# zrlhahaha/Direct12PBRRenderer

Measured on AMD Instinct MI355X. Metric: shaded Mpixel/s at 4K G-buffer (full deferred frame: clustered shade + bloom + auto-exposure + ACES), higher is better.
Workload: dtype f32

## Files before the change

### direct12pbrrenderer_amd/csrc/shade.hip

```cpp
#include <cstring>
#include <type_traits>
#include "pbr_internal.hpp"
#include "pbr_device.hpp"

using namespace pbr;

struct ShadeParams {
    pbr_sh_pack sh;
    float InvView[9];
    float CameraPos[3];
    float Near, Far;
    float near_width, near_height;
    float log_far_near;
    float inv_near, slice_k;
    uint32_t x0, y0, w, h, full_w, full_h;
    const uint32_t* A;
    const uint32_t* B;
    const uint32_t* C;
    const float* depth;
    const uint8_t* stencil;
    uint32_t pitch;
    const pbr_half* lut;
    uint32_t lut_res;
    const pbr_half* env;
    uint32_t env_size, env_mips;
    uint32_t env_mip_off[16];
    const pbr_cluster* clusters;
    const pbr_light* lights;
    pbr_half* hdr;
    uint32_t hdr_pitch;
    float* hdr_f32;
};

__device__ __forceinline__ float view_space_depth(float d, float near_z, float far_z) {
#pragma clang fp contract(off)
    const float range = far_z - near_z;
    const float prod = d * range;
    const float den = far_z - prod;
    const float num = near_z * far_z;
    return num / den;
}

__device__ __forceinline__ float view_space_depth_quick(float d, float near_z, float far_z) {
#pragma clang fp contract(off)
    const float range = far_z - near_z;
    const float prod = d * range;
    const float den = far_z - prod;
    return (near_z * far_z) * rcp(den);
}

__device__ __forceinline__ float sign_custom(float x) { return x < 0.0f ? -1.0f : 1.0f; }

__device__ __forceinline__ V3 decode_octahedron(float u, float v) {
    V3 d = v3(u * 2.0f - 1.0f, v * 2.0f - 1.0f, 0.0f);
    d.z = 1.0f - fabsf(d.x) - fabsf(d.y);
    if (d.z < 0.0f) {
// ... 31 lines not shown
struct ShadeRects {
    uint32_t n, rows_big, rows_small;
    uint32_t x0[SHADE_MAX_RECTS], y0[SHADE_MAX_RECTS], w[SHADE_MAX_RECTS], h[SHADE_MAX_RECTS];
    uint32_t cols[SHADE_MAX_RECTS], nb_big[SHADE_MAX_RECTS], first[SHADE_MAX_RECTS + 1];
};

constexpr int SHADE_BLOCK = 256;
constexpr int SHADE_ROWS = 8;
constexpr int MAX_STAGED_TILES = 12;
constexpr int LIST_STRIDE = 34;

typedef float f2 __attribute__((ext_vector_type(2)));
__device__ __forceinline__ f2 f2s(float a) { return f2{a, a}; }
__device__ __forceinline__ f2 max2(f2 a, f2 b) { return f2{fmaxf(a.x, b.x), fmaxf(a.y, b.y)}; }
typedef __attribute__((address_space(3))) const float lds_cf;
__device__ __forceinline__ f2 rsq2(f2 a) { return f2{rsq(a.x), rsq(a.y)}; }
__device__ __forceinline__ f2 rcp2(f2 a) { return f2{rcp(a.x), rcp(a.y)}; }

__device__ __forceinline__ f2 mul2_sat(f2 a, f2 b) {
    f2 r;
    asm("s_nop 0\n\tv_pk_mul_f32 %0, %1, %2 clamp\n\ts_nop 0" : "=v"(r) : "v"(a), "v"(b));
    return r;
}

__device__ __forceinline__ f2 zero2() {
    f2 r;
    asm("v_pk_mov_b32 %0, 0, 0\n\ts_nop 0" : "=v"(r));
    return r;
}

struct alignas(8) H4x2 { H4 a, b; };
struct alignas(4) H2x2 { H2 a, b; };

template <bool STAGED_LISTS, int LSTRIDE, bool F32OUT>
__device__ __forceinline__ void shade_pixel(const ShadeParams& p, const float* llds, const uint32_t* lists, const uint32_t* mip_off,
                                            int tile_x0, int tile_y0, int tiles_x, int n_lights, int q_safe, uint32_t px, uint32_t py, float4 row) {
    const uint32_t gi = __umul24(py, p.pitch) + px;
    auto at = [](const auto* base, uint32_t byte_off) { return *reinterpret_cast<std::remove_reference_t<decltype(*base)>*>(reinterpret_cast<const char*>(base) + byte_off); };
    if (at(p.stencil, gi) == 0) return;
    const float inv255 = 1.0f / 255.0f;

    const float u = ((float)(p.x0 + px) + 0.5f) / (float)p.full_w;
    V3 pos, view, n;
    float z_vs, roughness, depth_keep;
    {
        const uint32_t b = at(p.B, gi * 4u), c = at(p.C, gi * 4u);
        const float depth_ndc = at(p.depth, gi * 4u);
        const float ndc_x = 2.0f * u - 1.0f;
        const V3 cvv = v3(ndc_x * 0.5f * p.near_width, row.y, p.Near);
        const V3 camera_vec = v3(p.InvView[0] * cvv.x + p.InvView[1] * cvv.y + p.InvView[2] * cvv.z,
                                 p.InvView[3] * cvv.x + p.InvView[4] * cvv.y + p.InvView[5] * cvv.z,
                                 p.InvView[6] * cvv.x + p.InvView[7] * cvv.y + p.InvView[8] * cvv.z);
        roughness = (float)(c & 255u) * inv255;
        n = normalize3(decode_octahedron((float)(b & 255u) * inv255, (float)((b >> 8) & 255u) * inv255));
        z_vs = view_space_depth_quick(depth_ndc, p.Near, p.Far);
        depth_keep = depth_ndc;
        const V3 cam = v3(p.CameraPos[0], p.CameraPos[1], p.CameraPos[2]);
        const float zs = z_vs * p.inv_near;
        pos = v3(cam.x + camera_vec.x * zs, cam.y + camera_vec.y * zs, cam.z + camera_vec.z * zs);
        view = normalize3(cam - pos);
    }
    const float NdV = dot3(n, view);
    const float NdotV = fmaxf(NdV, 0.0f);

    float s1x = 0.0f, s1y = 0.0f, s1z = 0.0f, s2x = 0.0f, s2y = 0.0f, s2z = 0.0f, s3x = 0.0f, s3y = 0.0f, s3z = 0.0f;
#ifndef PBR_EXP_NOLOOP
    if (STAGED_LISTS || n_lights > 0) {
        int sx = (int)floorf(u * (float)PBR_CLUSTER_X);
        int sy = (int)row.z;
        float zc = fminf(fmaxf(z_vs, p.Near), p.Far);
        const float t_quick = p.slice_k * __builtin_amdgcn_logf(zc * p.inv_near);
        const float t_frac = t_quick - floorf(t_quick);
        int sz = (int)t_quick;
        if (__any(!(t_frac > 1.0e-4f && t_frac < 1.0f - 1.0e-4f))) {
            zc = fminf(fmaxf(view_space_depth(depth_keep, p.Near, p.Far), p.Near), p.Far);
            sz = (int)((float)PBR_CLUSTER_Z * logf(zc / p.Near) / p.log_far_near);
        }
        sx = clampi(sx, 0, PBR_CLUSTER_X - 1);
        sz = clampi(sz, 0, PBR_CLUSTER_Z - 1);
        const float ra = roughness * roughness;
        const float a4m1 = ra * ra - 1.0f;
        const float k = (roughness + 1.0f) * (roughness + 1.0f) * 0.125f;
        const float one_k = 1.0f - k;
        const float c4 = 4.0e4f * NdotV;
        const float t_floor = EPSILON_F * INV_PI_F;
        f2 a1x = zero2(), a1y = zero2(), a1z = zero2(), a2x = zero2(), a2y = zero2(), a2z = zero2(), a3x = zero2(), a3y = zero2(), a3z = zero2();
        const float att_c0 = llds[6 * LSTRIDE], att_c1 = llds[7 * LSTRIDE], att_c2 = llds[8 * LSTRIDE];
        auto light2 = [&](auto q_safe, auto t_safe, const lds_cf* la, const lds_cf* lb, auto att_uniform) {
            constexpr bool QSAFE = decltype(q_safe)::value, TSAFE = decltype(t_safe)::value, ATT = decltype(att_uniform)::value;
            auto comp = [&](int c) { return f2{la[c * LSTRIDE], lb[c * LSTRIDE]}; };
            const f2 dx = comp(0) - f2s(pos.x), dy = comp(1) - f2s(pos.y), dz = comp(2) - f2s(pos.z);
            const f2 d2 = dx * dx + dy * dy + dz * dz;
            const f2 invd = rsq2(d2);
            const f2 dn = dx * n.x + dy * n.y + dz * n.z;
            const f2 NdotL = mul2_sat(dn, invd);
            const f2 wx = dx * invd + f2s(view.x), wy = dy * invd + f2s(view.y), wz = dz * invd + f2s(view.z);
            const f2 h2 = wx * wx + (wy * wy + (wz * wz + f2s(1.0e-15f)));
            const f2 nw = dn * invd + f2s(NdV);
            const f2 tn = (nw * nw) * a4m1 + h2;
            const f2 h4 = h2 * h2;
            f2 Tn = tn * tn;
            if constexpr (!TSAFE) Tn = max2(Tn, h4 * t_floor);
            const f2 A = NdotL * one_k + f2s(k);
            f2 Q;
            if constexpr (ATT) Q = d2 * (invd * f2s(att_c1) + f2s(att_c2)) + f2s(att_c0);
            else Q = d2 * (invd * comp(7) + comp(8)) + comp(6);
            if constexpr (!QSAFE) Q = max2(Q, f2s(EPSILON_F));
            const f2 TA = Tn * A;
            const f2 r = rcp2(Q * TA);
            const f2 q = NdotL * r;
            const f2 X = q * TA;
            const f2 gs = mul2_sat(NdotL, f2s(c4));
            const f2 fm = f2s(1.0f) - NdotL;
            const f2 fm2 = fm * fm;
            const f2 f5 = fm2 * fm2 * fm;
            const f2 w2 = (q * gs) * h4;
            const f2 w1 = X - X * f5;
            const f2 w3 = w2 * f5;
            const f2 cr = comp(3), cg = comp(4), cb = comp(5);
            a1x += cr * w1; a1y += cg * w1; a1z += cb * w1;
            a2x += cr * w2; a2y += cg * w2; a2z += cb * w2;
            a3x += cr * w3; a3y += cg * w3; a3z += cb * w3;
        };
        const lds_cf* const ltab = (const lds_cf*)llds;
        if (STAGED_LISTS) {
            const uint32_t* my = lists + __mul24(__mul24(__mul24(sy - tile_y0, tiles_x) + (sx - tile_x0), PBR_CLUSTER_Z) + sz, LIST_STRIDE);
            const int nl = my[0];
            const bool t_ok = __all(ra * ra >= 6.0e-4f) != 0;
            auto walk = [&](auto qs, auto ts, auto au) {
                int i = 0;
                do {
                    const uint2 pair = *reinterpret_cast<const uint2*>(my + 2 + i);
                    light2(qs, ts, (const lds_cf*)(uintptr_t)pair.x, (const lds_cf*)(uintptr_t)pair.y, au);
                    i += 2;
                } while (i < nl);
            };
            if (q_safe & 1) {
                if (t_ok) { if (q_safe & 2) walk(std::true_type{}, std::true_type{}, std::true_type{}); else walk(std::true_type{}, std::true_type{}, std::false_type{}); }
                else if (q_safe & 2) walk(std::true_type{}, std::false_type{}, std::true_type{});
                else walk(std::true_type{}, std::false_type{}, std::false_type{});
            } else walk(std::false_type{}, std::false_type{}, std::false_type{});
        } else {
            const pbr_cluster* cl = p.clusters + (sz + sx * PBR_CLUSTER_Z + sy * PBR_CLUSTER_X * PBR_CLUSTER_Z);
            const int nl = min(max(cl->NumLights, 0), PBR_MAX_LIGHTS_PER_CLUSTER);
            auto idx = [&](int q) { return q < nl ? min(max(cl->LightIndex[q], 0), n_lights - 1) : n_lights; };
            for (int i = 0; i < nl; i += 2) light2(std::false_type{}, std::false_type{}, ltab + idx(i), ltab + idx(i + 1), std::false_type{});
        }
        s1x = a1x.x + a1x.y; s1y = a1y.x + a1y.y; s1z = a1z.x + a1z.y;
        s2x = a2x.x + a2x.y; s2y = a2y.x + a2y.y; s2z = a2z.x + a2z.y;
        s3x = a3x.x + a3x.y; s3y = a3y.x + a3y.y; s3z = a3z.x + a3z.y;
    }
#endif

    const uint32_t a = at(p.A, gi * 4u);
    const float metallic = (float)((at(p.C, gi * 4u) >> 8) & 255u) * inv255;
    const V3 albedo = v3((float)(a & 255u) * inv255, (float)((a >> 8) & 255u) * inv255, (float)((a >> 16) & 255u) * inv255);
    const float emission = (float)(a >> 24) * inv255;
    const V3 F0 = v3(0.04f + metallic * (albedo.x - 0.04f), 0.04f + metallic * (albedo.y - 0.04f), 0.04f + metallic * (albedo.z - 0.04f));
    V3 out;
    {
        const float ra = roughness * roughness;
        const float k = (roughness + 1.0f) * (roughness + 1.0f) * 0.125f;
        const float spec_pix = NdotV > 0.0f ? ra * ra * (0.25f * INV_PI_F) * rcp(fmaxf(NdotV * (1.0f - k) + k, EPSILON_F)) : 0.0f;
        const float kd = (1.0f - metallic) * INV_PI_F;
        out.x = (1.0f - F0.x) * (kd * albedo.x * s1x + spec_pix * s3x) + F0.x * spec_pix * s2x;
        out.y = (1.0f - F0.y) * (kd * albedo.y * s1y + spec_pix * s3y) + F0.y * spec_pix * s2y;
        out.z = (1.0f - F0.z) * (kd * albedo.z * s1z + spec_pix * s3z) + F0.z * spec_pix * s2z;
        out = out + albedo * emission;

#ifndef PBR_EXP_NOSH
        const float bx = n.x * n.y, by = n.y * n.z, bz = n.z * n.z, bw = n.z * n.x;
        const float cc = n.x * n.x - n.y * n.y;
        const pbr_sh_pack& s = p.sh;
        const float ir = (s.sha_r[0] * n.x + s.sha_r[1] * n.y + s.sha_r[2] * n.z + s.sha_r[3]) +
                         ((s.shb_r[0] * bx + s.shb_r[1] * by + s.shb_r[2] * bz + s.shb_r[3] * bw) + s.shc[0] * cc);
        const float ig = (s.sha_g[0] * n.x + s.sha_g[1] * n.y + s.sha_g[2] * n.z + s.sha_g[3]) +
                         ((s.shb_g[0] * bx + s.shb_g[1] * by + s.shb_g[2] * bz + s.shb_g[3] * bw) + s.shc[1] * cc);
        const float ib = (s.sha_b[0] * n.x + s.sha_b[1] * n.y + s.sha_b[2] * n.z + s.sha_b[3]) +
                         ((s.shb_b[0] * bx + s.shb_b[1] * by + s.shb_b[2] * bz + s.shb_b[3] * bw) + s.shc[2] * cc);
        out.x += albedo.x * kd * ir;
        out.y += albedo.y * kd * ig;
        out.z += albedo.z * kd * ib;
#endif
    }

#ifndef PBR_EXP_NOIBL
    {
#ifndef PBR_EXP_NOENV
        const V3 R = normalize3(n * (2.0f * NdV) - view);
        float lod = roughness * (float)PBR_ENV_MIPS;
        lod = snap8(fminf(fmaxf(lod, 0.0f), (float)(p.env_mips - 1)));
        const float fl = floorf(lod);
        const uint32_t l0 = (uint32_t)fl, l1 = min(l0 + 1, p.env_mips - 1);
        const float env_f = lod - fl;
        uint32_t face;
        float cu, cv;
        {
            const float ma = 0.5f * fabsf(__builtin_amdgcn_cubema(R.x, R.y, R.z));
            const float sc = __builtin_amdgcn_cubesc(R.x, R.y, R.z), tc = __builtin_amdgcn_cubetc(R.x, R.y, R.z);
            face = (uint32_t)__builtin_amdgcn_cubeid(R.x, R.y, R.z);
            const float inv = rcp(ma);
            cu = (sc * inv + 1.0f) * 0.5f;
            cv = (tc * inv + 1.0f) * 0.5f;
        }
        struct Foot { H4x2 r0, r1; float w00, w10, w01, w11; };
        auto foot = [&](uint32_t l, uint32_t mip_off, float wl) {
            const int s = (int)(p.env_size >> l), sq = s + 1;
            const float fxp = snap8(cu * (float)s) - 0.5f, fyp = snap8(cv * (float)s) - 0.5f;
            const float flx = floorf(fxp), fly = floorf(fyp);
            const float fx = fxp - flx, fy = fyp - fly;
            const uint32_t o = __umul24(__umul24(face, (uint32_t)sq) + (uint32_t)((int)fly + 1), (uint32_t)sq) + (uint32_t)((int)flx + 1);
            const char* q = reinterpret_cast<const char*>(p.env) + (mip_off + o * 4u) * 8u;
            Foot f;
            f.r0 = *reinterpret_cast<const H4x2*>(q);
            f.r1 = *reinterpret_cast<const H4x2*>(q + 16);
            const float wy1 = fy * wl, wy0 = wl - wy1;
            f.w10 = fx * wy0; f.w00 = wy0 - f.w10;
            f.w11 = fx * wy1; f.w01 = wy1 - f.w11;
            return f;
        };
        const Foot fa = foot(l0, mip_off[l0], 1.0f - env_f);
        const Foot fb = foot(l1, mip_off[l1], env_f);
        auto chan = [&](h16 a00, h16 a10, h16 a01, h16 a11, h16 b00, h16 b10, h16 b01, h16 b11) {
            float r = __builtin_fmaf((float)a00, fa.w00, 0.0f);
            r = __builtin_fmaf((float)a10, fa.w10, r);
            r = __builtin_fmaf((float)a01, fa.w01, r);
            r = __builtin_fmaf((float)a11, fa.w11, r);
            r = __builtin_fmaf((float)b00, fb.w00, r);
            r = __builtin_fmaf((float)b10, fb.w10, r);
            r = __builtin_fmaf((float)b01, fb.w01, r);
            return __builtin_fmaf((float)b11, fb.w11, r);
        };
        const V3 envc = v3(chan(fa.r0.a.x, fa.r0.b.x, fa.r1.a.x, fa.r1.b.x, fb.r0.a.x, fb.r0.b.x, fb.r1.a.x, fb.r1.b.x),
                           chan(fa.r0.a.y, fa.r0.b.y, fa.r1.a.y, fa.r1.b.y, fb.r0.a.y, fb.r0.b.y, fb.r1.a.y, fb.r1.b.y),
                           chan(fa.r0.a.z, fa.r0.b.z, fa.r1.a.z, fa.r1.b.z, fb.r0.a.z, fb.r0.b.z, fb.r1.a.z, fb.r1.b.z));
#else
        const V3 envc = v3(0.5f, 0.5f, 0.5f);
#endif
#ifndef PBR_EXP_NOLUT
        const int lr = (int)p.lut_res;
        const float lrf = (float)lr;
        const float xs = snap8(roughness * lrf) - 0.5f, ys = snap8(NdotV * lrf) - 0.5f;
        const float xfl = floorf(xs), yfl = floorf(ys);
        const int xi = (int)xfl, yi = (int)yfl;
        const int y0 = clampi(yi, 0, lr - 1), y1 = clampi(yi + 1, 0, lr - 1);
        const int xb = clampi(xi, 0, max(lr - 2, 0));
        const float fx = xi < 0 ? 0.0f : (xi > lr - 2 ? 1.0f : xs - xfl), fy = ys - yfl;
        const H2* lut = reinterpret_cast<const H2*>(p.lut);
        H2x2 lt0, lt1;
        if (lr > 1) {
            const char* lb8 = reinterpret_cast<const char*>(lut);
            lt0 = *reinterpret_cast<const H2x2*>(lb8 + (__umul24((uint32_t)y0, (uint32_t)lr) + (uint32_t)xb) * 4u);
            lt1 = *reinterpret_cast<const H2x2*>(lb8 + (__umul24((uint32_t)y1, (uint32_t)lr) + (uint32_t)xb) * 4u);
        } else {
            lt0.a = lt0.b = lut[0];
            lt1 = lt0;
        }
        const float wx0 = 1.0f - fx, wy0 = 1.0f - fy;
        auto xl = [&](h16 a, h16 b) { return __builtin_fmaf((float)b, fx, __builtin_fmaf((float)a, wx0, 0.0f)); };
        const float la = xl(lt0.a.x, lt0.b.x) * wy0 + xl(lt1.a.x, lt1.b.x) * fy;
        const float lb = xl(lt0.a.y, lt0.b.y) * wy0 + xl(lt1.a.y, lt1.b.y) * fy;
#else
        const float la = 0.5f, lb = 0.25f;
#endif
        out.x += envc.x * (F0.x * la + lb);
        out.y += envc.y * (F0.y * la + lb);
        out.z += envc.z * (F0.z * la + lb);
    }
#endif
    const uint32_t ho = __umul24(py, p.hdr_pitch) + px;
    if (F32OUT) *reinterpret_cast<float4*>(reinterpret_cast<char*>(p.hdr_f32) + ho * 16u) = make_float4(out.x, out.y, out.z, 1.0f);
    else store_h4(reinterpret_cast<pbr_half*>(reinterpret_cast<char*>(p.hdr) + ho * 8u), f4(out.x, out.y, out.z, 1.0f));
}

#ifdef PBR_SHADE_TIMING
__device__ unsigned long long g_shade_item_stamp[4 * 160000];
extern "C" int pbr_debug_shade_stamps(unsigned long long* blocks, int n_blocks, unsigned long long* items, int n_items) {
    (void)blocks; (void)n_blocks;
    return (int)hipMemcpyFromSymbol(items, HIP_SYMBOL(g_shade_item_stamp), sizeof(unsigned long long) * 4 * n_items);
}
extern "C" int pbr_debug_shade_stamps_reset() {
    void* i = nullptr;
    int e = (int)hipGetSymbolAddress(&i, HIP_SYMBOL(g_shade_item_stamp));
    if (e == 0) e = (int)hipMemset(i, 0, sizeof(g_shade_item_stamp));
    return e;
}
// ... 15 lines not shown
    const uint32_t* A;
    const uint32_t* B;
    const uint32_t* C;
    const float* depth;
    const uint8_t* stencil;
    const pbr_cluster* clusters;
    const pbr_light* lights;
    pbr_half* hdr;
    uint32_t pitch, hdr_pitch;
    int n_lights;
};
struct ShadeViews { ShadeView v[PBR_MAX_VIEWS]; };
static_assert(sizeof(ShadeParams) + sizeof(ShadeViews) + sizeof(ShadeRects) + 16 <= 4096 - 256, "k_deferred_shade<.., ShadeViews>: kernel arguments over 4 KiB");

template <bool STAGED_LISTS, int LSTRIDE, bool F32OUT, class VS = NoViews>
__global__ __launch_bounds__(SHADE_BLOCK, SHADE_MIN_WAVES) void k_deferred_shade(ShadeParams p_, int n_lights_, int max_clusters, ShadeRects rc, VS vs) {
    constexpr bool MV = !std::is_same_v<VS, NoViews>;
    ShadeParams q;
    int n_views_lights = 0;
    if constexpr (MV) {
        const ShadeView& v = vs.v[blockIdx.y];
        q = p_;
        for (int i = 0; i < 9; i++) q.InvView[i] = v.InvView[i];
        for (int i = 0; i < 3; i++) q.CameraPos[i] = v.CameraPos[i];
        q.Near = v.Near; q.Far = v.Far; q.near_width = v.near_width; q.near_height = v.near_height;
        q.log_far_near = v.log_far_near; q.inv_near = v.inv_near; q.slice_k = v.slice_k;
        q.A = v.A; q.B = v.B; q.C = v.C; q.depth = v.depth; q.stencil = v.stencil; q.pitch = v.pitch;
        q.clusters = v.clusters; q.lights = v.lights; q.hdr = v.hdr; q.hdr_pitch = v.hdr_pitch;
        n_views_lights = v.n_lights;
    }
    const ShadeParams& p = MV ? q : p_;
    const int n_lights = MV ? n_views_lights : n_lights_;
    extern __shared__ float4 lds_raw[];
    __shared__ uint32_t s_mip_off[16];
    const unsigned long long t_start = SHADE_NOW();
    (void)t_start;
    if (threadIdx.x < 16) s_mip_off[threadIdx.x] = p_.env_mip_off[threadIdx.x];
    float* llds = reinterpret_cast<float*>(lds_raw);
    uint32_t* lists = reinterpret_cast<uint32_t*>(llds + ((LIGHT_PLANES * LSTRIDE + 1) & ~1));
    int my_safe = 1, my_same = 1;
    const float att0 = n_lights > 0 ? p.lights[0].C0 : 1.0f, att1 = n_lights > 0 ? p.lights[0].C1 : 0.0f, att2 = n_lights > 0 ? p.lights[0].C2 : 0.0f;
    if (threadIdx.x == 0) {
        llds[0 * LSTRIDE + n_lights] = 1.0e15f; llds[1 * LSTRIDE + n_lights] = 1.0e15f; llds[2 * LSTRIDE + n_lights] = 1.0e15f;
        llds[3 * LSTRIDE + n_lights] = 0.0f; llds[4 * LSTRIDE + n_lights] = 0.0f; llds[5 * LSTRIDE + n_lights] = 0.0f;
        llds[6 * LSTRIDE + n_lights] = 1.0f; llds[7 * LSTRIDE + n_lights] = 0.0f; llds[8 * LSTRIDE + n_lights] = 0.0f;
    }
    for (int i = threadIdx.x; i < n_lights; i += SHADE_BLOCK) {
        const pbr_light l = p.lights[i];
        my_safe &= (l.C0 >= EPSILON_F) & (l.C1 >= 0.0f) & (l.C2 >= 0.0f);
        my_same &= (l.C0 == att0) & (l.C1 == att1) & (l.C2 == att2);
        llds[0 * LSTRIDE + i] = l.Position[0];
        llds[1 * LSTRIDE + i] = l.Position[1];
        llds[2 * LSTRIDE + i] = l.Position[2];
        llds[3 * LSTRIDE + i] = l.Color[0] * l.Intensity;
        llds[4 * LSTRIDE + i] = l.Color[1] * l.Intensity;
        llds[5 * LSTRIDE + i] = l.Color[2] * l.Intensity;
        llds[6 * LSTRIDE + i] = l.C0;
        llds[7 * LSTRIDE + i] = l.C1;
        llds[8 * LSTRIDE + i] = l.C2;
    }
    uint32_t r = 0;
    while (r + 1 < rc.n && blockIdx.x >= rc.first[r + 1]) r++;
    const uint32_t lb = blockIdx.x - rc.first[r];
    const uint32_t bx0 = rc.x0[r] + (lb % rc.cols[r]) * SHADE_BLOCK, x_end = rc.x0[r] + rc.w[r];
    const uint32_t by = lb / rc.cols[r], nb_big = rc.nb_big[r], rows_big = rc.rows_big, rows_small = rc.rows_small;
    const uint32_t y_begin = rc.y0[r] + (by < nb_big ? by * rows_big : nb_big * rows_big + (by - nb_big) * rows_small);
    const uint32_t y_end = min(y_begin + (by < nb_big ? rows_big : rows_small), rc.y0[r] + rc.h[r]);
    int tile_x0 = 0, tile_y0 = 0, tiles_x = 1;
    const uint32_t lds_base = (uint32_t)(uintptr_t)(lds_cf*)llds;
    if (STAGED_LISTS) {
        const uint32_t bx1 = min(bx0 + SHADE_BLOCK, x_end) - 1;
        auto tx = [&](uint32_t x) { return clampi((int)floorf((((float)(p.x0 + x) + 0.5f) / (float)p.full_w) * (float)PBR_CLUSTER_X), 0, PBR_CLUSTER_X - 1); };
// ... 11 lines not shown
            const int part = threadIdx.x & 7;
            const float inv_tiles_x = rcp((float)tiles_x);
            for (int c = threadIdx.x >> 3; c < n_cl; c += SHADE_BLOCK / 8) {
                const int z = c & 7, t = c >> 3;
                const int ty_ = (int)(((float)t + 0.5f) * inv_tiles_x), cx = tile_x0 + (t - ty_ * tiles_x), cy = tile_y0 + ty_;
                const pbr_cluster* cl = p.clusters + (z + cx * PBR_CLUSTER_Z + cy * PBR_CLUSTER_X * PBR_CLUSTER_Z);
                const int cnt = n_lights > 0 ? min(max(cl->NumLights, 0), PBR_MAX_LIGHTS_PER_CLUSTER) : 0;
                const Idx4 v = *reinterpret_cast<const Idx4*>(cl->LightIndex + 4 * part);
                uint32_t* l = lists + c * LIST_STRIDE;
                if (4 * part < max(cnt, 2)) {
                    auto entry = [&](int k, int raw) { return lds_base + 4u * (uint32_t)(4 * part + k < cnt ? min(max(raw, 0), n_lights - 1) : n_lights); };
                    uint2* e = reinterpret_cast<uint2*>(l + 2 + 4 * part);
                    e[0] = make_uint2(entry(0, v.x), entry(1, v.y));
                    e[1] = make_uint2(entry(2, v.z), entry(3, v.w));
                }
                if (part == 0) *reinterpret_cast<uint2*>(l) = make_uint2((uint32_t)max((cnt + 1) & ~1, 2), 0u);
            }
        }
    }
    __shared__ float4 s_row[SHADE_ROWS];
    if (threadIdx.x < (uint32_t)SHADE_ROWS) {
        const float v = ((float)(p.y0 + y_begin + threadIdx.x) + 0.5f) / (float)p.full_h;
        const float ndc_y = 1.0f - 2.0f * v;
        s_row[threadIdx.x] = make_float4(v, ndc_y * 0.5f * p.near_height, (float)clampi((int)floorf((1.0f - v) * (float)PBR_CLUSTER_Y), 0, PBR_CLUSTER_Y - 1), 0.0f);
    }
    const int q_safe = (__syncthreads_and(my_safe) != 0 ? 1 : 0) | (__syncthreads_and(my_same) != 0 ? 2 : 0);
    SHADE_ISTAMP(blockIdx.x, 0, t_start);
    SHADE_ISTAMP(blockIdx.x, 1, SHADE_NOW());
    SHADE_ISTAMP(blockIdx.x, 3, ((unsigned long long)(y_end - y_begin) << 48) | blockIdx.x);
    const uint32_t px = bx0 + threadIdx.x;
#ifndef PBR_SHADE_TIMING
    if (px >= x_end) return;
    for (uint32_t py = y_begin; py < y_end; py++)
        shade_pixel<STAGED_LISTS, LSTRIDE, F32OUT>(p, llds, lists, s_mip_off, tile_x0, tile_y0, tiles_x, n_lights, q_safe, px, py, s_row[py - y_begin]);
#else
    if (px < x_end)
        for (uint32_t py = y_begin; py < y_end; py++)
            shade_pixel<STAGED_LISTS, LSTRIDE, F32OUT>(p, llds, lists, s_mip_off, tile_x0, tile_y0, tiles_x, n_lights, q_safe, px, py, s_row[py - y_begin]);
    SHADE_ISTAMP_MAX(blockIdx.x, 2, SHADE_NOW());
#endif
}

extern "C" {

pbr_status pbr_env_pad(pbr_ctx* ctx, const pbr_half* env, uint32_t size, uint32_t mips, pbr_half* out_padded) {
    if (!ctx) return PBR_ERR_INVALID;
    PBR_REQUIRE(ctx, env && out_padded, "pbr_env_pad: null pointer");
    PBR_REQUIRE(ctx, size >= 1 && size <= 8192 && mips >= 1 && mips <= 16 && (size >> (mips - 1)) >= 1, "pbr_env_pad: bad size/mips");
    for (uint32_t m = 0; m < mips; m++) {
        const int s = (int)(size >> m);
        const size_t n = (size_t)6 * (s + 1) * (s + 1) * 4;
        hipLaunchKernelGGL(k_env_pad, dim3((unsigned)((n + 255) / 256)), dim3(256), 0, ctx->stream,
                           env + 4 * cube_mip_offset(size, m), out_padded + 4 * env_padded_mip_offset(size, m), s);
        pbr_status r = launched(ctx, "k_env_pad");
        if (r) return r;
    }
    return PBR_OK;
}

}

static void camera_params(const pbr_global* g, ShadeParams& p) {
    p.sh = g->SkyBoxSH;
    for (int r = 0; r < 3; r++)
        for (int c = 0; c < 3; c++) p.InvView[r * 3 + c] = g->InvView[r * 4 + c];
    for (int i = 0; i < 3; i++) p.CameraPos[i] = g->CameraPos[i];
    p.Near = g->Near; p.Far = g->Far;
    p.near_height = 2.0f * g->Near * tanf(g->Fov / 2.0f);
    p.near_width = p.near_height * g->Ratio;
    p.log_far_near = logf(g->Far / g->Near);
    p.inv_near = (float)(1.0 / (double)g->Near);
    p.slice_k = (float)((double)PBR_CLUSTER_Z / log2((double)g->Far / (double)g->Near));
}

static ShadeParams shade_params(const pbr_global* g, const pbr_half* lut, uint32_t lut_res, const pbr_half* env, uint32_t env_size, uint32_t env_mips) {
    ShadeParams p{};
    camera_params(g, p);
    p.lut = lut; p.lut_res = lut_res; p.env = env; p.env_size = env_size; p.env_mips = env_mips;
    for (uint32_t m = 0; m < 16; m++) p.env_mip_off[m] = (uint32_t)env_padded_mip_offset(env_size, m < env_mips ? m : env_mips - 1);
    return p;
}

static const char* shade_tables_bad(const pbr_half* lut, uint32_t lut_res, const pbr_half* env, uint32_t env_size, uint32_t env_mips) {
    if (!lut || !env) return "null pointer";
    if (!(lut_res >= 1 && env_size >= 1 && env_mips >= 1 && env_mips <= 16 && (env_size >> (env_mips - 1)) >= 1)) return "bad LUT/env size";
    if (!(lut_res <= 16384 && (uint64_t)pbr_env_padded_texels(env_size, env_mips) * 8u < (1ull << 32)))
        return "LUT larger than 16384^2 or padded env chain of 4 GiB or more (32-bit texture offsets)";
    if (((uintptr_t)env & 7u) != 0 || ((uintptr_t)lut & 3u) != 0) return "env must be 8-byte and lut 4-byte aligned";
    return nullptr;
}

static const char* shade_target_bad(const pbr_global* g, const pbr_gbuffer& gb, const pbr_cluster* clusters, const void* out, uint32_t out_pitch,
                                    uint32_t w, uint32_t h, const pbr_light* lights, int num_lights) {
    if (!clusters || !out) return "null pointer";
    if (!(gb.A && gb.B && gb.C && gb.depth && gb.stencil)) return "null G-buffer plane";
    if (!(gb.pitch >= w && out_pitch >= w)) return "pitch < width";
    if (!((uint64_t)gb.pitch * h * 4u < (1ull << 32) && (uint64_t)out_pitch * h * 16u < (1ull << 32)))
        return "target too large for 32-bit plane offsets (pitch x rows x 16 bytes must stay below 4 GiB)";
    if (!(g->Near > 0.0f && g->Far > g->Near)) return "need 0 < Near < Far";
    if (!(num_lights >= 0 && num_lights <= PBR_MAX_SCENE_LIGHTS)) return "light count out of [0, 1024]";
    if (!(num_lights == 0 || lights != nullptr)) return "null lights";
    return nullptr;
}

static ShadeRects shade_schedule(const pbr_ctx* ctx, const uint32_t (*rects)[4], uint32_t n_rects, uint32_t n_views) {
    static const float big_frac = pbr::knob_float("PBR_SHADE_BIGFRAC", 0.92f);
    static const uint32_t rows_small_cfg = (uint32_t)pbr::knob_int("PBR_SHADE_ROWS_SMALL", 1);
    static const uint32_t rows_big_cfg = (uint32_t)pbr::knob_int("PBR_SHADE_ROWS_BIG", 0);
    const uint32_t rows_small = rows_small_cfg >= 1 && rows_small_cfg <= (uint32_t)SHADE_ROWS ? rows_small_cfg : 1u;
    uint64_t row_segments = 0;
    for (uint32_t r = 0; r < n_rects; r++) row_segments += (uint64_t)((rects[r][2] + SHADE_BLOCK - 1) / SHADE_BLOCK) * rects[r][3];
    row_segments *= n_views;
    uint32_t rows_big = (uint32_t)SHADE_ROWS;
    const uint64_t slots = (uint64_t)ctx->cu_count * SHADE_MIN_WAVES;
    if (row_segments * 10 < slots * 13 * SHADE_ROWS) {
        const uint32_t rws = (uint32_t)((row_segments * 10 + slots * 8) / (slots * 16));
        rows_big = rws < 2 ? 2u : (rws > (uint32_t)SHADE_ROWS ? (uint32_t)SHADE_ROWS : rws);
    }
    if (rows_big_cfg >= 1 && rows_big_cfg <= (uint32_t)SHADE_ROWS) rows_big = rows_big_cfg;
    ShadeRects rc{};
    rc.n = n_rects; rc.rows_big = rows_big; rc.rows_small = rows_small < rows_big ? rows_small : rows_big;
    uint32_t blocks = 0;
    for (uint32_t r = 0; r < n_rects; r++) {
        const uint32_t* q = rects[r];
        rc.x0[r] = q[0]; rc.y0[r] = q[1]; rc.w[r] = q[2]; rc.h[r] = q[3];
        rc.cols[r] = (q[2] + SHADE_BLOCK - 1) / SHADE_BLOCK;
        rc.nb_big[r] = (uint32_t)((float)(q[3] / rows_big) * fminf(fmaxf(big_frac, 0.0f), 1.0f));
        const uint32_t rest = q[3] - rc.nb_big[r] * rows_big;
        rc.first[r] = blocks;
        blocks += rc.cols[r] * (rc.nb_big[r] + (rest + rc.rows_small - 1) / rc.rows_small);
    }
    rc.first[n_rects] = blocks;
    return rc;
}

template <bool F32OUT, class VS>
static pbr_status shade_dispatch(pbr_ctx* ctx, const ShadeParams& p, int num_lights, int max_lights, const ShadeRects& rc, uint32_t n_views, const VS& vs) {
    const uint32_t span_x = (uint32_t)((uint64_t)(SHADE_BLOCK - 1) * PBR_CLUSTER_X / p.full_w) + 2;
    const uint32_t span_y = (uint32_t)((uint64_t)(SHADE_ROWS - 1) * PBR_CLUSTER_Y / p.full_h) + 2;
    const int lstride = max_lights <= 256 ? 257 : PBR_MAX_SCENE_LIGHTS + 1;
    const size_t plane_bytes = (size_t)((LIGHT_PLANES * lstride + 1) & ~1) * sizeof(float);
    const bool staged = span_x * span_y <= (uint32_t)MAX_STAGED_TILES &&
                        plane_bytes + (size_t)span_x * span_y * PBR_CLUSTER_Z * LIST_STRIDE * sizeof(uint32_t) <= 65536;
    const int max_clusters = staged ? (int)(span_x * span_y) * PBR_CLUSTER_Z : 0;
    const size_t lds = plane_bytes + (size_t)max_clusters * LIST_STRIDE * sizeof(uint32_t);
    const dim3 grid(rc.first[rc.n], n_views), blk(SHADE_BLOCK);
    if (staged && lstride == 257) hipLaunchKernelGGL((k_deferred_shade<true, 257, F32OUT, VS>), grid, blk, lds, ctx->stream, p, num_lights, max_clusters, rc, vs);
    else if (staged) hipLaunchKernelGGL((k_deferred_shade<true, PBR_MAX_SCENE_LIGHTS + 1, F32OUT, VS>), grid, blk, lds, ctx->stream, p, num_lights, max_clusters, rc, vs);
    else if (lstride == 257) hipLaunchKernelGGL((k_deferred_shade<false, 257, F32OUT, VS>), grid, blk, lds, ctx->stream, p, num_lights, 0, rc, vs);
    else hipLaunchKernelGGL((k_deferred_shade<false, PBR_MAX_SCENE_LIGHTS + 1, F32OUT, VS>), grid, blk, lds, ctx->stream, p, num_lights, 0, rc, vs);
    return launched(ctx, std::is_same_v<VS, NoViews> ? "k_deferred_shade" : "k_deferred_shade<views>");
}

template <bool F32OUT>
static pbr_status shade_launch(pbr_ctx* ctx, const pbr_global* g, const pbr_tile* tile, const pbr_gbuffer* gb,
                               const pbr_half* lut, uint32_t lut_res,
                               const pbr_half* env, uint32_t env_size, uint32_t env_mips,
                               const pbr_cluster* clusters, const pbr_light* lights, int num_lights,
                               pbr_half* hdr, float* hdr_f32, uint32_t hdr_pitch,
                               const uint32_t (*rects)[4] = nullptr, uint32_t n_rects = 0) {
    if (!ctx) return PBR_ERR_INVALID;
    const char* who = "pbr_deferred_shade";
    PBR_REQUIRE(ctx, g && tile && gb, "pbr_deferred_shade: null pointer");
    PBR_REQUIRE(ctx, tile->w >= 1 && tile->h >= 1 && tile->w <= 65535 && tile->h <= 65535, "pbr_deferred_shade: bad tile size");
    PBR_REQUIRE(ctx, tile->x0 + tile->w <= tile->full_w && tile->y0 + tile->h <= tile->full_h, "pbr_deferred_shade: tile outside frame");
    PBR_CHECK(ctx, who, shade_target_bad(g, *gb, clusters, F32OUT ? (const void*)hdr_f32 : (const void*)hdr, hdr_pitch, tile->w, tile->h, lights, num_lights));
    PBR_CHECK(ctx, who, shade_tables_bad(lut, lut_res, env, env_size, env_mips));
    const uint32_t whole[1][4] = {{0, 0, tile->w, tile->h}};
    if (!rects) { rects = whole; n_rects = 1; }
    PBR_REQUIRE(ctx, n_rects >= 1 && n_rects <= (uint32_t)SHADE_MAX_RECTS, "pbr_deferred_shade: 1 .. 5 rectangles");
    for (uint32_t r = 0; r < n_rects; r++) {
        const uint32_t* q = rects[r];
        PBR_REQUIRE(ctx, q[2] >= 1 && q[3] >= 1 && q[0] + q[2] <= tile->w && q[1] + q[3] <= tile->h, "pbr_deferred_shade: rectangle outside the tile");
    }
    ShadeParams p = shade_params(g, lut, lut_res, env, env_size, env_mips);
    p.x0 = tile->x0; p.y0 = tile->y0; p.w = tile->w; p.h = tile->h; p.full_w = tile->full_w; p.full_h = tile->full_h;
    p.A = gb->A; p.B = gb->B; p.C = gb->C; p.depth = gb->depth; p.stencil = gb->stencil; p.pitch = gb->pitch;
    p.clusters = clusters; p.lights = lights; p.hdr = hdr; p.hdr_pitch = hdr_pitch; p.hdr_f32 = hdr_f32;
    return shade_dispatch<F32OUT>(ctx, p, num_lights, num_lights, shade_schedule(ctx, rects, n_rects, 1), 1, NoViews{});
}

extern "C" {

pbr_status pbr_deferred_shade(pbr_ctx* ctx, const pbr_global* g, const pbr_tile* tile, const pbr_gbuffer* gb,
                              const pbr_half* lut, uint32_t lut_res,
                              const pbr_half* env, uint32_t env_size, uint32_t env_mips,
                              const pbr_cluster* clusters, const pbr_light* lights, int num_lights,
                              pbr_half* hdr, uint32_t hdr_pitch) {
    return shade_launch<false>(ctx, g, tile, gb, lut, lut_res, env, env_size, env_mips, clusters, lights, num_lights, hdr, nullptr, hdr_pitch);
}

pbr_status pbr_deferred_shade_rects(pbr_ctx* ctx, const pbr_global* g, const pbr_tile* tile, const pbr_gbuffer* gb,
                                    const pbr_half* lut, uint32_t lut_res,
                                    const pbr_half* env, uint32_t env_size, uint32_t env_mips,
                                    const pbr_cluster* clusters, const pbr_light* lights, int num_lights,
                                    pbr_half* hdr, uint32_t hdr_pitch, const uint32_t (*rects)[4], uint32_t n_rects) {
    if (ctx && !rects) return pbr::fail(ctx, PBR_ERR_INVALID, "pbr_deferred_shade_rects: null rectangle list");
    return shade_launch<false>(ctx, g, tile, gb, lut, lut_res, env, env_size, env_mips, clusters, lights, num_lights, hdr, nullptr, hdr_pitch, rects, n_rects);
}

pbr_status pbr_deferred_shade_f32(pbr_ctx* ctx, const pbr_global* g, const pbr_tile* tile, const pbr_gbuffer* gb,
                                  const pbr_half* lut, uint32_t lut_res,
                                  const pbr_half* env, uint32_t env_size, uint32_t env_mips,
                                  const pbr_cluster* clusters, const pbr_light* lights, int num_lights,
                                  float* hdr_f32, uint32_t hdr_pitch) {
    if (ctx && hdr_f32 && ((uintptr_t)hdr_f32 & 15u) != 0) return pbr::fail(ctx, PBR_ERR_INVALID, "pbr_deferred_shade_f32: output must be 16-byte aligned");
    return shade_launch<true>(ctx, g, tile, gb, lut, lut_res, env, env_size, env_mips, clusters, lights, num_lights, nullptr, hdr_f32, hdr_pitch);
}

pbr_status pbr_deferred_shade_views(pbr_ctx* ctx, const pbr_view* views, uint32_t n, uint32_t w, uint32_t h,
                                    const pbr_half* lut, uint32_t lut_res,
                                    const pbr_half* env, uint32_t env_size, uint32_t env_mips) {
    if (!ctx) return PBR_ERR_INVALID;
    const char* who = "pbr_deferred_shade_views";
    PBR_REQUIRE(ctx, views_count_ok(views, n), "pbr_deferred_shade_views: need 1 .. PBR_MAX_VIEWS views");
    PBR_REQUIRE(ctx, w >= 1 && h >= 1 && w <= 65535 && h <= 65535, "pbr_deferred_shade_views: bad frame size");
    PBR_CHECK(ctx, who, shade_tables_bad(lut, lut_res, env, env_size, env_mips));
    ShadeViews vs{};
    int max_lights = 0;
    for (uint32_t i = 0; i < n; i++) {
        const pbr_view& v = views[i];
        PBR_CHECK(ctx, who, shade_target_bad(&v.g, v.gb, v.clusters, v.hdr, v.hdr_pitch, w, h, v.lights, v.num_lights));
        PBR_REQUIRE(ctx, memcmp(&v.g.SkyBoxSH, &views[0].g.SkyBoxSH, sizeof(pbr_sh_pack)) == 0, "pbr_deferred_shade_views: SkyBoxSH differs between views");
        ShadeParams c;
        camera_params(&v.g, c);
        ShadeView& d = vs.v[i];
        for (int k = 0; k < 9; k++) d.InvView[k] = c.InvView[k];
        for (int k = 0; k < 3; k++) d.CameraPos[k] = c.CameraPos[k];
        d.Near = c.Near; d.Far = c.Far; d.near_width = c.near_width; d.near_height = c.near_height;
        d.log_far_near = c.log_far_near; d.inv_near = c.inv_near; d.slice_k = c.slice_k;
        d.A = v.gb.A; d.B = v.gb.B; d.C = v.gb.C; d.depth = v.gb.depth; d.stencil = v.gb.stencil; d.pitch = v.gb.pitch;
        d.clusters = v.clusters; d.lights = v.lights; d.hdr = v.hdr; d.hdr_pitch = v.hdr_pitch; d.n_lights = v.num_lights;
        max_lights = v.num_lights > max_lights ? v.num_lights : max_lights;
    }
    PBR_REQUIRE(ctx, views_disjoint(views, n, 1, [&](const pbr_view& v, int, uintptr_t& lo, uintptr_t& hi) {
                    lo = addr(v.hdr); hi = lo + ((size_t)v.hdr_pitch * (h - 1) + w) * 8u; }),
                "pbr_deferred_shade_views: two views share an HDR target");
    ShadeParams p = shade_params(&views[0].g, lut, lut_res, env, env_size, env_mips);
    p.w = p.full_w = w; p.h = p.full_h = h;
    const uint32_t whole[1][4] = {{0, 0, w, h}};
    return shade_dispatch<false>(ctx, p, 0, max_lights, shade_schedule(ctx, whole, 1, n), n, vs);
}

}
```

Baseline: 17530.

## Precompute per-roughness-code shading constants into an LDS lookup table

Each block fills a 256-entry LDS table, one entry per 8-bit roughness code, holding the GGX constants, environment mip footprint parameters and the LUT x offset and weight. Per-pixel shading reads these from LDS instead of recomputing roughness-derived values and env LOD math. The extra 12 KB of LDS per block can lower occupancy, so the scheduler now derives blocks per CU from the actual LDS footprint. Each block also pays a small setup fill.

```diff
diff --git a/direct12pbrrenderer_amd/csrc/shade.hip b/direct12pbrrenderer_amd/csrc/shade.hip
--- a/direct12pbrrenderer_amd/csrc/shade.hip
+++ b/direct12pbrrenderer_amd/csrc/shade.hip
@@ -22,6 +22,7 @@
     uint32_t pitch;
     const pbr_half* lut;
     uint32_t lut_res;
+    float lut_res_f;
     const pbr_half* env;
     uint32_t env_size, env_mips;
     uint32_t env_mip_off[16];
@@ -119,8 +120,51 @@
 struct alignas(8) H4x2 { H4 a, b; };
 struct alignas(4) H2x2 { H2 a, b; };
 
+struct alignas(16) RoughEntry {
+    float env_f, a4m1, k, spec_c;
+    float sf0; uint32_t sq0, off0, lut_xoff;
+    float sf1; uint32_t sq1, off1; float lut_fx;
+};
+static_assert(sizeof(RoughEntry) == 48, "RoughEntry: three 16-byte words");
+enum { RE_ENV_F = 0, RE_A4M1 = 1, RE_K = 2, RE_SPEC = 3, RE_LUT_XOFF = 7, RE_LUT_FX = 11 };
+constexpr int ROUGH_CODES = 256;
+__host__ __device__ constexpr uint32_t rough_table_offset(int lstride, int max_clusters) {
+    return ((uint32_t)(((LIGHT_PLANES * lstride + 1) & ~1) + max_clusters * LIST_STRIDE) * 4u + 15u) & ~15u;
+}
+static_assert(ROUGH_CODES == 256, "one entry per UNORM8 code; one thread of the block fills each");
+
+__device__ __forceinline__ RoughEntry rough_entry_fill(uint32_t code, uint32_t lut_res, uint32_t env_size, uint32_t env_mips, const uint32_t* mip_off) {
+#pragma clang fp contract(off)
+    RoughEntry e;
+    const float inv255 = 1.0f / 255.0f;
+    const float cf = (float)code;
+    const float roughness = cf * inv255;
+    const float ra = roughness * roughness;
+    const float ra2 = ra * ra;
+    e.a4m1 = __builtin_fmaf(ra, ra, -1.0f);
+    const float r1 = __builtin_fmaf(cf, inv255, 1.0f);
+    e.k = (r1 * r1) * 0.125f;
+    const float spec_c = ra2 * (0.25f * INV_PI_F);
+    e.spec_c = ra2 >= 6.0e-4f ? -spec_c : spec_c;
+    float lod = roughness * (float)PBR_ENV_MIPS;
+    lod = snap8(fminf(fmaxf(lod, 0.0f), (float)(env_mips - 1)));
+    const float fl = floorf(lod);
+    const uint32_t l0 = (uint32_t)fl, l1 = min(l0 + 1, env_mips - 1);
+    e.env_f = lod - fl;
+    const int s0 = (int)(env_size >> l0), s1 = (int)(env_size >> l1);
+    e.sf0 = (float)s0; e.sq0 = (uint32_t)(s0 + 1); e.off0 = mip_off[l0] * 8u;
+    e.sf1 = (float)s1; e.sq1 = (uint32_t)(s1 + 1); e.off1 = mip_off[l1] * 8u;
+    const int lr = (int)lut_res;
+    const float xs = snap8(roughness * (float)lr) - 0.5f;
+    const float xfl = floorf(xs);
+    const int xi = (int)xfl;
+    e.lut_xoff = (uint32_t)clampi(xi, 0, max(lr - 2, 0)) * 4u;
+    e.lut_fx = xi < 0 ? 0.0f : (xi > lr - 2 ? 1.0f : xs - xfl);
+    return e;
+}
+
 template <bool STAGED_LISTS, int LSTRIDE, bool F32OUT>
-__device__ __forceinline__ void shade_pixel(const ShadeParams& p, const float* llds, const uint32_t* lists, const uint32_t* mip_off,
+__device__ __forceinline__ void shade_pixel(const ShadeParams& p, const float* llds, const uint32_t* lists, const RoughEntry* rtab,
                                             int tile_x0, int tile_y0, int tiles_x, int n_lights, int q_safe, uint32_t px, uint32_t py, float4 row) {
     const uint32_t gi = __umul24(py, p.pitch) + px;
     auto at = [](const auto* base, uint32_t byte_off) { return *reinterpret_cast<std::remove_reference_t<decltype(*base)>*>(reinterpret_cast<const char*>(base) + byte_off); };
@@ -129,7 +173,8 @@
 
     const float u = ((float)(p.x0 + px) + 0.5f) / (float)p.full_w;
     V3 pos, view, n;
-    float z_vs, roughness, depth_keep;
+    float z_vs, depth_keep;
+    const lds_cf* re;
     {
         const uint32_t b = at(p.B, gi * 4u), c = at(p.C, gi * 4u);
         const float depth_ndc = at(p.depth, gi * 4u);
@@ -138,7 +183,7 @@
         const V3 camera_vec = v3(p.InvView[0] * cvv.x + p.InvView[1] * cvv.y + p.InvView[2] * cvv.z,
                                  p.InvView[3] * cvv.x + p.InvView[4] * cvv.y + p.InvView[5] * cvv.z,
                                  p.InvView[6] * cvv.x + p.InvView[7] * cvv.y + p.InvView[8] * cvv.z);
-        roughness = (float)(c & 255u) * inv255;
+        re = (const lds_cf*)reinterpret_cast<const float*>(rtab) + (c & 255u) * (uint32_t)(sizeof(RoughEntry) / 4);
         n = normalize3(decode_octahedron((float)(b & 255u) * inv255, (float)((b >> 8) & 255u) * inv255));
         z_vs = view_space_depth_quick(depth_ndc, p.Near, p.Far);
         depth_keep = depth_ndc;
@@ -165,9 +210,7 @@
         }
         sx = clampi(sx, 0, PBR_CLUSTER_X - 1);
         sz = clampi(sz, 0, PBR_CLUSTER_Z - 1);
-        const float ra = roughness * roughness;
-        const float a4m1 = ra * ra - 1.0f;
-        const float k = (roughness + 1.0f) * (roughness + 1.0f) * 0.125f;
+        const float a4m1 = re[RE_A4M1], k = re[RE_K], t_flag = re[RE_SPEC];
         const float one_k = 1.0f - k;
         const float c4 = 4.0e4f * NdotV;
         const float t_floor = EPSILON_F * INV_PI_F;
@@ -213,7 +256,7 @@
         if (STAGED_LISTS) {
             const uint32_t* my = lists + __mul24(__mul24(__mul24(sy - tile_y0, tiles_x) + (sx - tile_x0), PBR_CLUSTER_Z) + sz, LIST_STRIDE);
             const int nl = my[0];
-            const bool t_ok = __all(ra * ra >= 6.0e-4f) != 0;
+            const bool t_ok = __all(__float_as_int(t_flag) < 0) != 0;
             auto walk = [&](auto qs, auto ts, auto au) {
                 int i = 0;
                 do {
@@ -246,9 +289,9 @@
     const V3 F0 = v3(0.04f + metallic * (albedo.x - 0.04f), 0.04f + metallic * (albedo.y - 0.04f), 0.04f + metallic * (albedo.z - 0.04f));
     V3 out;
     {
-        const float ra = roughness * roughness;
-        const float k = (roughness + 1.0f) * (roughness + 1.0f) * 0.125f;
-        const float spec_pix = NdotV > 0.0f ? ra * ra * (0.25f * INV_PI_F) * rcp(fmaxf(NdotV * (1.0f - k) + k, EPSILON_F)) : 0.0f;
+        asm volatile("" : "+v"(re));
+        const float k = re[RE_K];
+        const float spec_pix = NdotV > 0.0f ? fabsf(re[RE_SPEC]) * rcp(fmaxf(NdotV * (1.0f - k) + k, EPSILON_F)) : 0.0f;
         const float kd = (1.0f - metallic) * INV_PI_F;
         out.x = (1.0f - F0.x) * (kd * albedo.x * s1x + spec_pix * s3x) + F0.x * spec_pix * s2x;
         out.y = (1.0f - F0.y) * (kd * albedo.y * s1y + spec_pix * s3y) + F0.y * spec_pix * s2y;
@@ -275,11 +318,10 @@
     {
 #ifndef PBR_EXP_NOENV
         const V3 R = normalize3(n * (2.0f * NdV) - view);
-        float lod = roughness * (float)PBR_ENV_MIPS;
-        lod = snap8(fminf(fmaxf(lod, 0.0f), (float)(p.env_mips - 1)));
-        const float fl = floorf(lod);
-        const uint32_t l0 = (uint32_t)fl, l1 = min(l0 + 1, p.env_mips - 1);
-        const float env_f = lod - fl;
+        const float env_f = re[RE_ENV_F];
+        typedef float f4v __attribute__((ext_vector_type(4)));
+        typedef __attribute__((address_space(3))) const f4v lds_cf4;
+        const f4v lv0 = reinterpret_cast<lds_cf4*>(re)[1], lv1 = reinterpret_cast<lds_cf4*>(re)[2];
         uint32_t face;
         float cu, cv;
         {
@@ -291,13 +333,12 @@
             cv = (tc * inv + 1.0f) * 0.5f;
         }
         struct Foot { H4x2 r0, r1; float w00, w10, w01, w11; };
-        auto foot = [&](uint32_t l, uint32_t mip_off, float wl) {
-            const int s = (int)(p.env_size >> l), sq = s + 1;
-            const float fxp = snap8(cu * (float)s) - 0.5f, fyp = snap8(cv * (float)s) - 0.5f;
+        auto foot = [&](float sf, uint32_t sq, uint32_t level_off, float wl) {
+            const float fxp = snap8(cu * sf) - 0.5f, fyp = snap8(cv * sf) - 0.5f;
             const float flx = floorf(fxp), fly = floorf(fyp);
             const float fx = fxp - flx, fy = fyp - fly;
-            const uint32_t o = __umul24(__umul24(face, (uint32_t)sq) + (uint32_t)((int)fly + 1), (uint32_t)sq) + (uint32_t)((int)flx + 1);
-            const char* q = reinterpret_cast<const char*>(p.env) + (mip_off + o * 4u) * 8u;
+            const uint32_t o = __umul24(__umul24(face, sq) + (uint32_t)((int)fly + 1), sq) + (uint32_t)((int)flx + 1);
+            const char* q = reinterpret_cast<const char*>(p.env) + (level_off + o * 32u);
             Foot f;
             f.r0 = *reinterpret_cast<const H4x2*>(q);
             f.r1 = *reinterpret_cast<const H4x2*>(q + 16);
@@ -306,8 +347,8 @@
             f.w11 = fx * wy1; f.w01 = wy1 - f.w11;
             return f;
         };
-        const Foot fa = foot(l0, mip_off[l0], 1.0f - env_f);
-        const Foot fb = foot(l1, mip_off[l1], env_f);
+        const Foot fa = foot(lv0.x, __float_as_uint(lv0.y), __float_as_uint(lv0.z), 1.0f - env_f);
+        const Foot fb = foot(lv1.x, __float_as_uint(lv1.y), __float_as_uint(lv1.z), env_f);
         auto chan = [&](h16 a00, h16 a10, h16 a01, h16 a11, h16 b00, h16 b10, h16 b01, h16 b11) {
             float r = __builtin_fmaf((float)a00, fa.w00, 0.0f);
             r = __builtin_fmaf((float)a10, fa.w10, r);
@@ -326,19 +367,24 @@
 #endif
 #ifndef PBR_EXP_NOLUT
         const int lr = (int)p.lut_res;
-        const float lrf = (float)lr;
-        const float xs = snap8(roughness * lrf) - 0.5f, ys = snap8(NdotV * lrf) - 0.5f;
-        const float xfl = floorf(xs), yfl = floorf(ys);
-        const int xi = (int)xfl, yi = (int)yfl;
+        const float lrf = p.lut_res_f;
+        const float ys = snap8(NdotV * lrf) - 0.5f;
+        const float yfl = floorf(ys);
+        const int yi = (int)yfl;
         const int y0 = clampi(yi, 0, lr - 1), y1 = clampi(yi + 1, 0, lr - 1);
-        const int xb = clampi(xi, 0, max(lr - 2, 0));
-        const float fx = xi < 0 ? 0.0f : (xi > lr - 2 ? 1.0f : xs - xfl), fy = ys - yfl;
+#ifndef PBR_EXP_NOENV
+        const uint32_t xoff = __float_as_uint(lv0.w);
+        const float fx = lv1.w, fy = ys - yfl;
+#else
+        const uint32_t xoff = __float_as_uint(re[RE_LUT_XOFF]);
+        const float fx = re[RE_LUT_FX], fy = ys - yfl;
+#endif
         const H2* lut = reinterpret_cast<const H2*>(p.lut);
         H2x2 lt0, lt1;
         if (lr > 1) {
             const char* lb8 = reinterpret_cast<const char*>(lut);
-            lt0 = *reinterpret_cast<const H2x2*>(lb8 + (__umul24((uint32_t)y0, (uint32_t)lr) + (uint32_t)xb) * 4u);
-            lt1 = *reinterpret_cast<const H2x2*>(lb8 + (__umul24((uint32_t)y1, (uint32_t)lr) + (uint32_t)xb) * 4u);
+            lt0 = *reinterpret_cast<const H2x2*>(lb8 + (__umul24((uint32_t)y0, (uint32_t)lr) * 4u + xoff));
+            lt1 = *reinterpret_cast<const H2x2*>(lb8 + (__umul24((uint32_t)y1, (uint32_t)lr) * 4u + xoff));
         } else {
             lt0.a = lt0.b = lut[0];
             lt1 = lt0;
@@ -420,12 +466,13 @@
     const ShadeParams& p = MV ? q : p_;
     const int n_lights = MV ? n_views_lights : n_lights_;
     extern __shared__ float4 lds_raw[];
-    __shared__ uint32_t s_mip_off[16];
     const unsigned long long t_start = SHADE_NOW();
     (void)t_start;
-    if (threadIdx.x < 16) s_mip_off[threadIdx.x] = p_.env_mip_off[threadIdx.x];
     float* llds = reinterpret_cast<float*>(lds_raw);
     uint32_t* lists = reinterpret_cast<uint32_t*>(llds + ((LIGHT_PLANES * LSTRIDE + 1) & ~1));
+    static_assert(SHADE_BLOCK == ROUGH_CODES, "one thread fills one roughness entry");
+    RoughEntry* rtab = reinterpret_cast<RoughEntry*>(reinterpret_cast<char*>(lds_raw) + rough_table_offset(LSTRIDE, max_clusters));
+    rtab[threadIdx.x] = rough_entry_fill(threadIdx.x, p_.lut_res, p_.env_size, p_.env_mips, p_.env_mip_off);
     int my_safe = 1, my_same = 1;
     const float att0 = n_lights > 0 ? p.lights[0].C0 : 1.0f, att1 = n_lights > 0 ? p.lights[0].C1 : 0.0f, att2 = n_lights > 0 ? p.lights[0].C2 : 0.0f;
     if (threadIdx.x == 0) {
@@ -503,11 +550,11 @@
 #ifndef PBR_SHADE_TIMING
     if (px >= x_end) return;
     for (uint32_t py = y_begin; py < y_end; py++)
-        shade_pixel<STAGED_LISTS, LSTRIDE, F32OUT>(p, llds, lists, s_mip_off, tile_x0, tile_y0, tiles_x, n_lights, q_safe, px, py, s_row[py - y_begin]);
+        shade_pixel<STAGED_LISTS, LSTRIDE, F32OUT>(p, llds, lists, rtab, tile_x0, tile_y0, tiles_x, n_lights, q_safe, px, py, s_row[py - y_begin]);
 #else
     if (px < x_end)
         for (uint32_t py = y_begin; py < y_end; py++)
-            shade_pixel<STAGED_LISTS, LSTRIDE, F32OUT>(p, llds, lists, s_mip_off, tile_x0, tile_y0, tiles_x, n_lights, q_safe, px, py, s_row[py - y_begin]);
+            shade_pixel<STAGED_LISTS, LSTRIDE, F32OUT>(p, llds, lists, rtab, tile_x0, tile_y0, tiles_x, n_lights, q_safe, px, py, s_row[py - y_begin]);
     SHADE_ISTAMP_MAX(blockIdx.x, 2, SHADE_NOW());
 #endif
 }
@@ -547,7 +594,7 @@
 static ShadeParams shade_params(const pbr_global* g, const pbr_half* lut, uint32_t lut_res, const pbr_half* env, uint32_t env_size, uint32_t env_mips) {
     ShadeParams p{};
     camera_params(g, p);
-    p.lut = lut; p.lut_res = lut_res; p.env = env; p.env_size = env_size; p.env_mips = env_mips;
+    p.lut = lut; p.lut_res = lut_res; p.lut_res_f = (float)lut_res; p.env = env; p.env_size = env_size; p.env_mips = env_mips;
     for (uint32_t m = 0; m < 16; m++) p.env_mip_off[m] = (uint32_t)env_padded_mip_offset(env_size, m < env_mips ? m : env_mips - 1);
     return p;
 }
@@ -574,7 +621,25 @@
     return nullptr;
 }
 
-static ShadeRects shade_schedule(const pbr_ctx* ctx, const uint32_t (*rects)[4], uint32_t n_rects, uint32_t n_views) {
+struct ShadeLds { int lstride, max_clusters; bool staged; size_t bytes; uint32_t blocks_per_cu; };
+static ShadeLds shade_lds(uint32_t full_w, uint32_t full_h, int max_lights) {
+    ShadeLds l{};
+    const uint32_t span_x = (uint32_t)((uint64_t)(SHADE_BLOCK - 1) * PBR_CLUSTER_X / full_w) + 2;
+    const uint32_t span_y = (uint32_t)((uint64_t)(SHADE_ROWS - 1) * PBR_CLUSTER_Y / full_h) + 2;
+    l.lstride = max_lights <= 256 ? 257 : PBR_MAX_SCENE_LIGHTS + 1;
+    const size_t table_bytes = (size_t)ROUGH_CODES * sizeof(RoughEntry);
+    l.staged = span_x * span_y <= (uint32_t)MAX_STAGED_TILES &&
+               rough_table_offset(l.lstride, (int)(span_x * span_y) * PBR_CLUSTER_Z) + table_bytes <= 65536;
+    l.max_clusters = l.staged ? (int)(span_x * span_y) * PBR_CLUSTER_Z : 0;
+    l.bytes = rough_table_offset(l.lstride, l.max_clusters) + table_bytes;
+    constexpr size_t LDS_PER_CU = 160 * 1024, LDS_GRANULE = 1280, STATIC_LDS = sizeof(float4) * SHADE_ROWS;
+    const size_t alloc = (l.bytes + STATIC_LDS + LDS_GRANULE - 1) / LDS_GRANULE * LDS_GRANULE;
+    const size_t fit = LDS_PER_CU / alloc;
+    l.blocks_per_cu = (uint32_t)(fit < (size_t)SHADE_MIN_WAVES ? (fit < 1 ? 1 : fit) : (size_t)SHADE_MIN_WAVES);
+    return l;
+}
+
+static ShadeRects shade_schedule(const pbr_ctx* ctx, const ShadeLds& lds, const uint32_t (*rects)[4], uint32_t n_rects, uint32_t n_views) {
     static const float big_frac = pbr::knob_float("PBR_SHADE_BIGFRAC", 0.92f);
     static const uint32_t rows_small_cfg = (uint32_t)pbr::knob_int("PBR_SHADE_ROWS_SMALL", 1);
     static const uint32_t rows_big_cfg = (uint32_t)pbr::knob_int("PBR_SHADE_ROWS_BIG", 0);
@@ -583,7 +648,7 @@
     for (uint32_t r = 0; r < n_rects; r++) row_segments += (uint64_t)((rects[r][2] + SHADE_BLOCK - 1) / SHADE_BLOCK) * rects[r][3];
     row_segments *= n_views;
     uint32_t rows_big = (uint32_t)SHADE_ROWS;
-    const uint64_t slots = (uint64_t)ctx->cu_count * SHADE_MIN_WAVES;
+    const uint64_t slots = (uint64_t)ctx->cu_count * lds.blocks_per_cu;
     if (row_segments * 10 < slots * 13 * SHADE_ROWS) {
         const uint32_t rws = (uint32_t)((row_segments * 10 + slots * 8) / (slots * 16));
         rows_big = rws < 2 ? 2u : (rws > (uint32_t)SHADE_ROWS ? (uint32_t)SHADE_ROWS : rws);
@@ -606,15 +671,10 @@
 }
 
 template <bool F32OUT, class VS>
-static pbr_status shade_dispatch(pbr_ctx* ctx, const ShadeParams& p, int num_lights, int max_lights, const ShadeRects& rc, uint32_t n_views, const VS& vs) {
-    const uint32_t span_x = (uint32_t)((uint64_t)(SHADE_BLOCK - 1) * PBR_CLUSTER_X / p.full_w) + 2;
-    const uint32_t span_y = (uint32_t)((uint64_t)(SHADE_ROWS - 1) * PBR_CLUSTER_Y / p.full_h) + 2;
-    const int lstride = max_lights <= 256 ? 257 : PBR_MAX_SCENE_LIGHTS + 1;
-    const size_t plane_bytes = (size_t)((LIGHT_PLANES * lstride + 1) & ~1) * sizeof(float);
-    const bool staged = span_x * span_y <= (uint32_t)MAX_STAGED_TILES &&
-                        plane_bytes + (size_t)span_x * span_y * PBR_CLUSTER_Z * LIST_STRIDE * sizeof(uint32_t) <= 65536;
-    const int max_clusters = staged ? (int)(span_x * span_y) * PBR_CLUSTER_Z : 0;
-    const size_t lds = plane_bytes + (size_t)max_clusters * LIST_STRIDE * sizeof(uint32_t);
+static pbr_status shade_dispatch(pbr_ctx* ctx, const ShadeParams& p, int num_lights, const ShadeLds& l, const ShadeRects& rc, uint32_t n_views, const VS& vs) {
+    const bool staged = l.staged;
+    const int lstride = l.lstride, max_clusters = l.max_clusters;
+    const size_t lds = l.bytes;
     const dim3 grid(rc.first[rc.n], n_views), blk(SHADE_BLOCK);
     if (staged && lstride == 257) hipLaunchKernelGGL((k_deferred_shade<true, 257, F32OUT, VS>), grid, blk, lds, ctx->stream, p, num_lights, max_clusters, rc, vs);
     else if (staged) hipLaunchKernelGGL((k_deferred_shade<true, PBR_MAX_SCENE_LIGHTS + 1, F32OUT, VS>), grid, blk, lds, ctx->stream, p, num_lights, max_clusters, rc, vs);
@@ -648,7 +708,8 @@
     p.x0 = tile->x0; p.y0 = tile->y0; p.w = tile->w; p.h = tile->h; p.full_w = tile->full_w; p.full_h = tile->full_h;
     p.A = gb->A; p.B = gb->B; p.C = gb->C; p.depth = gb->depth; p.stencil = gb->stencil; p.pitch = gb->pitch;
     p.clusters = clusters; p.lights = lights; p.hdr = hdr; p.hdr_pitch = hdr_pitch; p.hdr_f32 = hdr_f32;
-    return shade_dispatch<F32OUT>(ctx, p, num_lights, num_lights, shade_schedule(ctx, rects, n_rects, 1), 1, NoViews{});
+    const ShadeLds l = shade_lds(p.full_w, p.full_h, num_lights);
+    return shade_dispatch<F32OUT>(ctx, p, num_lights, l, shade_schedule(ctx, l, rects, n_rects, 1), 1, NoViews{});
 }
 
 extern "C" {
@@ -710,7 +771,8 @@
     ShadeParams p = shade_params(&views[0].g, lut, lut_res, env, env_size, env_mips);
     p.w = p.full_w = w; p.h = p.full_h = h;
     const uint32_t whole[1][4] = {{0, 0, w, h}};
-    return shade_dispatch<false>(ctx, p, 0, max_lights, shade_schedule(ctx, whole, 1, n), n, vs);
-}
-
-}
+    const ShadeLds l = shade_lds(w, h, max_lights);
+    return shade_dispatch<false>(ctx, p, 0, l, shade_schedule(ctx, l, whole, 1, n), n, vs);
+}
+
+}
```

After: 17590 (median of 6 runs). Within noise of the previous version (+0.4%).
